# trflorian/s3od

Hardware: AMD Instinct MI355X
Metric: train images/sec (dinob 1024px bf16) at 1/2/4/8 GPU; infer masks/sec 1GPU (higher is better)
Workload: dtype bf16; 1 GPU; synth_sod train model=dinob 1024px bs=16/GPU fwd+focal_iou loss+bwd+AdamW; model=dinob (DINOv3 ViT-B/16 + DPT + 3-mask head), global_batch=16, image_size=1024, parallelism=dp1, rccl_world_size=1

## Files before the change

s3od_amd/csrc/gemm.hpp:

```cpp
#pragma once
#include "common.hpp"
#include <algorithm>

constexpr int GEMM_THREADS = 512;
constexpr int GEMM_WAVES = GEMM_THREADS / 64;
template <typename T> struct KT { static constexpr int BK = 64; };
template <> struct KT<float> { static constexpr int BK = 32; };

DEV int kc_off(int r, int byte) { return r * 128 + ((((byte >> 4) ^ ((r >> 1) & 7)) << 4) | (byte & 15)); }
template <int RB> DEV int mc_off(int k, int byte) {
  constexpr int SLOTS = RB / 32;
  int g = ((k & 3) | (((k >> 3) & 1) << 2)) & (SLOTS - 1);
  return k * RB + ((((byte >> 5) ^ g) << 5) | (byte & 31));
}

struct ConvGeo {
  int B;
  int SH, SW, SC;
  int RH, RW;
  int KH, KW, s, p;
  int py, px, kh0, kw0, nth, ntw, qy0, qx0;
};

static inline ConvGeo make_class(ConvGeo g, int OH, int OW, int py, int px) {
// ... 819 lines not shown
      }
    };
    const int spr_ = BN / 8;
    if (fixed_cols && BM % (NT / spr_) == 0) {
      const int rpi = NT / spr_, cs = tid % spr_, r0 = tid / spr_, n = n0 + cs * 8, nit = BM / rpi;
      if (n < N) {
        dispatch([&](auto ACTC) {
#pragma unroll
          for (int it0 = 0; it0 < nit; it0 += EB) {
            __builtin_amdgcn_sched_barrier(0);
            float av[EB][8];
            Row8<TR> q[EB];
            long orow[EB];
#pragma unroll
            for (int u = 0; u < EB; u++) {
              const int it = it0 + u, r = r0 + it * rpi, m = m0 + r;
              if (it < nit) {
                const float4* src = (const float4*)(ct + r * LDT + cs * 8);
                const float4 x0 = src[0], x1 = src[1];
                av[u][0] = x0.x; av[u][1] = x0.y; av[u][2] = x0.z; av[u][3] = x0.w;
                av[u][4] = x1.x; av[u][5] = x1.y; av[u][6] = x1.z; av[u][7] = x1.w;
                orow[u] = m < M ? rm.map(m) : 0;
                if (res1) q[u].load(res1 + orow[u] * ldr1 + n);
              }
            }
#pragma unroll
            for (int u = 0; u < EB; u++) {
              const int it = it0 + u;
              if (it < nit && m0 + r0 + it * rpi < M) {
                float r1v[8];
                q[u].get(r1v);
                seg(ACTC, orow[u], n, av[u], r1v, b8, s8, h8);
              }
            }
          }
        });
      }
    } else {
      dispatch([&](auto ACTC) {
        for_segments(ct, LDT, BM, BN, m0, n0, M, N, tid, NT, [&](int m, int n, const float* a, int, int) {
          float av[8], bb[8], ss[8], hh[8], r1v[8];
#pragma unroll
          for (int e = 0; e < 8; e++) {
            av[e] = a[e];
            bb[e] = bias ? bias[n + e] : 0.f; ss[e] = scale ? scale[n + e] : 1.f; hh[e] = shift ? shift[n + e] : 0.f;
            r1v[e] = 0.f;
          }
          const long orow = rm.map(m);
          if (res1) load8<TR>(res1 + orow * ldr1 + n, r1v);
          seg(ACTC, orow, n, av, r1v, bb, ss, hh);
        });
      });
    }
    if (stats) {
      const int nph = NT / BN;
      const int c = tid % BN, ph = tid / BN;
      const int n = n0 + c;
      if (n < N) {
        float s = 0.f, q = 0.f;
        const float bn_ = bias ? bias[n] : 0.f;
        for (int r = ph; r < BM; r += nph) {
          if (m0 + r >= M) break;
          const float v = ct[r * LDT + c] + bn_;
          s += v; q += v * v;
        }
        const int rep = (int)(((unsigned)(blockIdx.y * gridDim.x + blockIdx.x) * (unsigned)nph + ph + (m0 / BM)) % S3OD_NREP);
        double* st = stats + (long)rep * 2 * N;
        atomicAdd(st + n, (double)s);
        atomicAdd(st + N + n, (double)q);
      }
    }
    if (csum) {
      lds_barrier();
      float* red = (float*)ct;
#pragma unroll
      for (int e = 0; e < 8; e++) red[tid * 8 + e] = cs8[e];
      lds_barrier();
      const int spr = BN / 8, nph = NT / spr;
      if (tid < BN && n0 + tid < N) {
        const int g = tid >> 3, e = tid & 7;
        float s = 0.f;
        for (int ph = 0; ph < nph; ph++) s += red[(ph * spr + g) * 8 + e];
        atomicAdd(csum + n0 + tid, s);
      }
    }
  }
};

struct EpiWgrad {
  float* dw; int M, N, Cx, taps;
  DEV void prepare(int) {}
  DEV void operator()(const float* ct, int LDT, int m0, int n0, int tid, int BM, int BN, int NT) const {
    const int total = BM * BN;
    for (int s = tid; s < total; s += NT) {
      int r = s / BN, c = s - r * BN;
      int m = m0 + r, n = n0 + c;
      if (m < M && n < N) {
        int tap = n / Cx, cin = n - tap * Cx;
        atomicAdd(dw + ((long)m * Cx + cin) * taps + tap, ct[r * LDT + c]);
      }
    }
  }
};

struct EpiWgradPart {
  float* ws; int M, N;
  int z = 0;
  DEV void prepare(int zz) { z = zz; }
  DEV void operator()(const float* ct, int LDT, int m0, int n0, int tid, int BM, int BN, int NT) const {
    float* slab = ws + (long)z * M * N;
    for_segments(ct, LDT, BM, BN, m0, n0, M, N, tid, NT, [&](int m, int n, const float* a, int, int) {
      float4* d = (float4*)(slab + (long)m * N + n);
      d[0] = make_float4(a[0], a[1], a[2], a[3]);
      d[1] = make_float4(a[4], a[5], a[6], a[7]);
    });
  }
};

template <bool KCL> struct PPFrag;
template <> struct PPFrag<true> {
  int o[2];
  DEV void init(int lane, int) {
#pragma unroll
    for (int kk = 0; kk < 2; kk++) o[kk] = kc_off(lane & 15, kk * 64 + (lane >> 4) * 16);
  }
  DEV bf16x8 read(const char* img, int row0, int kk) const { return *(const bf16x8*)(img + o[kk] + row0 * 128); }
};
template <> struct PPFrag<false> {
  int base, gk;
  DEV void init(int lane, int h64) {
    const int g = lane >> 4, i = lane & 15, q = i >> 2, p = i & 3;
    base = (8 * g + q) * 256 + 8 * p; gk = (q | ((g & 1) << 2)) ^ (h64 << 2);
  }
  DEV bf16x8 read(const char* img, int row0, int kk) const {
    typedef __attribute__((address_space(3))) s16x4 lds_s4;
    const char* a = img + base + ((((row0 >> 4) ^ gk)) << 5) + kk * 8192;
    s16x4 lo = __builtin_amdgcn_ds_read_tr16_b64_v4i16((lds_s4*)a);
    s16x4 hi = __builtin_amdgcn_ds_read_tr16_b64_v4i16((lds_s4*)(a + 1024));
    bf16x4 x = __builtin_bit_cast(bf16x4, lo), y = __builtin_bit_cast(bf16x4, hi);
    bf16x8 r;
    r[0] = x[0]; r[1] = x[1]; r[2] = x[2]; r[3] = x[3]; r[4] = y[0]; r[5] = y[1]; r[6] = y[2]; r[7] = y[3];
    return r;
  }
};


#ifdef S3OD_TIMELINE
static __device__ unsigned long long* s3od_tl;
#define S3OD_TL(slot, v) do { if (s3od_tl && threadIdx.x == 0) s3od_tl[((long)blockIdx.z * gridDim.y * gridDim.x + \
    blockIdx.y * gridDim.x + blockIdx.x) * 8 + (slot)] = (v); } while (0)
#else
#define S3OD_TL(slot, v) do { } while (0)
#endif

DEV void tile_of_block(int G, int& mt, int& nt) {
  const int nN = gridDim.x, nM = gridDim.y, nwg = nN * nM;
  const int L = blockIdx.y * nN + blockIdx.x;
  const int q = nwg >> 3, r = nwg & 7, xcd = L & 7, idx = L >> 3;
  const int W = (xcd < r ? xcd * (q + 1) : r * (q + 1) + (xcd - r) * q) + idx;
  if (G <= 0) { mt = W / nN; nt = W % nN; return; }
  const int per = G * nN, g = W / per, w = W - g * per, m_first = g * G, gs = min(nM - m_first, G);
  mt = m_first + w % gs; nt = w / gs;
}

template <class LA, class LB, class EPI>
__global__ void __launch_bounds__(GEMM_THREADS, 1) igemm_pp_kernel(LA la0, LB lb0, EPI epi, int KTILES, int split, int flags) {
  typedef bf16 T;
  constexpr int BM = 256, BN = 256, HB = 128 * 128, STG = 4 * HB, LDT = BN + 4;
  static_assert(sizeof(T) == 2 && KT<T>::BK == 64, "ping-pong kernel is bf16 only");
  static_assert(128 * LDT * 4 <= 160 * 1024 && 2 * STG <= 128 * LDT * 4, "ping-pong LDS budget");
  extern __shared__ __attribute__((aligned(16))) char smem[];
  const int tid = threadIdx.x, lane = tid & 63, wave = wave_id();
  const int wr = wave >> 2, wc = wave & 3;
  S3OD_TL(0, __builtin_amdgcn_s_memrealtime());
  S3OD_TL(3, ((unsigned long long)__builtin_amdgcn_s_getreg((20 << 0) | (0 << 6) | (31 << 11)) << 32) |
             (unsigned)__builtin_amdgcn_s_getreg((4 << 0) | (0 << 6) | (31 << 11)));
  int m0, n0;
  {
    int mt, nt_;
    tile_of_block((flags >> 8) & 0xff, mt, nt_);
    m0 = mt * BM; n0 = nt_ * BN;
  }
  const int per = (KTILES + split - 1) / split;
  const int kt0 = blockIdx.z * per, kt1 = min(KTILES, kt0 + per);
  const int nt = kt1 - kt0;
  epi.prepare(blockIdx.z);
  LA la1 = la0; LB lb1 = lb0;
  la0.setup(m0, tid); la1.setup(m0 + 128, tid);
  lb0.setup(n0, tid); lb1.setup(n0 + 128, tid);
  constexpr int NA = LA::NIW * 2;
  const bool stag = !(flags & 1);
  f32x4 acc[8][4];
#pragma unroll
  for (int i = 0; i < 8; i++)
#pragma unroll
    for (int j = 0; j < 4; j++) acc[i][j] = f32x4{0.f, 0.f, 0.f, 0.f};
  if (nt > 0) {
    la0.issue(kt0, smem); la1.issue(kt0, smem + HB); lb0.issue(kt0, smem + 2 * HB); lb1.issue(kt0, smem + 3 * HB);
    if (nt > 1) { la0.issue(kt0 + 1, smem + STG); la1.issue(kt0 + 1, smem + STG + HB); wait_vmcnt<NA>(); }
    else wait_vmcnt<0>();
    raw_barrier();
    if (wr && stag) raw_barrier();
    PPFrag<LA::KCL> pfa; pfa.init(lane, 0);
    PPFrag<LB::KCL> pfb; pfb.init(lane, wc & 1);
    const int boff = LB::KCL ? (wc & 1) * 64 * 128 : 0;
    bf16x8 fa[2][4][2], fb[2][2][2];
    auto rdA = [&](const char* As, int qm) {
#pragma unroll
      for (int i = 0; i < 4; i++)
#pragma unroll
        for (int kk = 0; kk < 2; kk++) {
          fa[qm][i][kk] = pfa.read(As, qm * 64 + i * 16, kk);
          if constexpr (LA::RELU) fa[qm][i][kk] = relu_frag(fa[qm][i][kk]);
        }
    };
    auto rdB = [&](const char* Bs, int qn) {
#pragma unroll
      for (int j = 0; j < 2; j++)
#pragma unroll
        for (int kk = 0; kk < 2; kk++) {
          fb[qn][j][kk] = pfb.read(Bs, qn * 32 + j * 16, kk);
          if constexpr (LB::RELU) fb[qn][j][kk] = relu_frag(fb[qn][j][kk]);
        }
    };
    auto mm = [&](int qm, int qn) {
      raw_barrier();
      wait_lgkm0();
      __builtin_amdgcn_s_setprio(1);
#pragma unroll
      for (int kk = 0; kk < 2; kk++)
#pragma unroll
        for (int i = 0; i < 4; i++)
#pragma unroll
          for (int j = 0; j < 2; j++)
            acc[qm * 4 + i][qn * 2 + j] =
                __builtin_amdgcn_mfma_f32_16x16x32_bf16(fb[qn][j][kk], fa[qm][i][kk], acc[qm * 4 + i][qn * 2 + j], 0, 0, 0);
      __builtin_amdgcn_s_setprio(0);
      raw_barrier();
    };
    for (int t = 0; t < nt; ++t) {
      char* cb = smem + (t & 1) * STG;
      char* nb = smem + ((t + 1) & 1) * STG;
      const char* As = cb + wr * HB;
      const char* Bs = cb + (2 + (wc >> 1)) * HB + boff;
      rdA(As, 0); rdB(Bs, 0);
      if (t + 1 < nt) lb0.issue(kt0 + t + 1, nb + 2 * HB);
      mm(0, 0);
      rdB(Bs, 1); rdA(As, 1);
      if (t + 1 < nt) lb1.issue(kt0 + t + 1, nb + 3 * HB);
      mm(0, 1);
      if (t + 2 < nt) la0.issue(kt0 + t + 2, cb);
      mm(1, 1);
      if (t + 2 < nt) { la1.issue(kt0 + t + 2, cb + HB); wait_vmcnt<NA>(); }
      else if (t + 1 < nt) wait_vmcnt<0>();
      mm(1, 0);
    }
    if (!wr && stag) raw_barrier();
  }
  S3OD_TL(1, __builtin_amdgcn_s_memrealtime());
  vm_drain();
  float* ct0 = (float*)smem;
  float* ct1 = ct0 + 64 * LDT;
  auto round = [&](auto CC) {
    constexpr int c = decltype(CC)::value;
    lds_barrier();
    {
      float* dst = wr ? ct1 : ct0;
#pragma unroll
      for (int i = 0; i < 4; i++)
#pragma unroll
        for (int j = 0; j < 4; j++) {
          const int r = i * 16 + (lane & 15), col = wc * 64 + j * 16 + (lane >> 4) * 4;
          *(f32x4*)(dst + r * LDT + col) = acc[c * 4 + i][j];
        }
    }
    lds_barrier();
    S3OD_TL(4 + 2 * c, __builtin_amdgcn_s_memrealtime());
#ifdef S3OD_TIMELINE
    if constexpr (std::is_same_v<EPI, EpiStd<bf16, bf16, bf16>>) {
      if (flags & 2) {
        const int cs = tid % 32, r0 = tid / 32;
#pragma unroll
        for (int it = 0; it < 8; it++) {
          const int r = r0 + (it & 3) * 16;
          const float* src_ = (it < 4 ? ct0 : ct1) + r * LDT + cs * 8;
          const float4 a = ((const float4*)src_)[0], b = ((const float4*)src_)[1];
          const float v[8] = {a.x, a.y, a.z, a.w, b.x, b.y, b.z, b.w};
          store8<bf16>(epi.out + (long)(m0 + (it < 4 ? 0 : 128) + c * 64 + r) * epi.ldo + n0 + cs * 8, v);
        }
        return;
      }
    }
#endif
    epi(ct0, LDT, m0 + c * 64, n0, tid, 64, BN, GEMM_THREADS);
    epi(ct1, LDT, m0 + 128 + c * 64, n0, tid, 64, BN, GEMM_THREADS);
    if (c == 0) S3OD_TL(5, __builtin_amdgcn_s_memrealtime());
  };
  round(std::integral_constant<int, 0>{});
  round(std::integral_constant<int, 1>{});
  S3OD_TL(2, __builtin_amdgcn_s_memrealtime());
}
constexpr int PP_LDS = 128 * (256 + 4) * 4;

template <class LA, class LB, class EPI>
int launch_igemm_q(LA la, LB lb, EPI epi, int M, int N, int KTILES, int split, int zdim_extra, hipStream_t st);

template <typename T, int BM, int BN, class LA, class LB, class EPI, int NST = 3, int WM_ = 0>
static int launch_igemm(LA la, LB lb, EPI epi, int M, int N, int KTILES, int split, int zdim_extra, hipStream_t st) {
  if constexpr (WM_ < 0) {
    static_assert(BM == 256 && BN == 256 && sizeof(T) == 2, "q config");
    return launch_igemm_q(la, lb, epi, M, N, KTILES, split, zdim_extra, st);
  } else if constexpr (LA::ROWS * 2 == BM) {
    static_assert(BM == 256 && BN == 256 && LB::ROWS == 128 && sizeof(T) == 2, "ping-pong config");
    if (!la.buf_ok() || !lb.buf_ok()) {
      s3od_set_error("igemm: operand window too large for a buffer descriptor or gather channels < %d", KT<T>::BK / 2);
      return 22;
    }
    auto kfn = igemm_pp_kernel<LA, LB, EPI>;
    static const bool attr = ((void)hipFuncSetAttribute((const void*)kfn, hipFuncAttributeMaxDynamicSharedMemorySize, PP_LDS), true);
    (void)attr;
    const int flags = S3OD_KNOB("S3OD_PP_FLAGS", 0) | (S3OD_KNOB("S3OD_GEMM_GROUP", 0) & 0xff) << 8;
    dim3 grid(cdiv(N, BN), cdiv(M, BM), split * zdim_extra);
    hipLaunchKernelGGL(kfn, grid, dim3(GEMM_THREADS), PP_LDS, st, la, lb, epi, KTILES, split, flags);
    return s3od_check_launch("igemm_pp");
  } else {
    if (!la.buf_ok() || !lb.buf_ok()) {
      s3od_set_error("igemm: operand window too large for a buffer descriptor or gather channels < %d", KT<T>::BK / 2);
      return 22;
    }
    typedef GemmShape<T, BM, BN, NST, WM_> S;
    auto kfn = igemm_kernel<T, BM, BN, NST, LA, LB, EPI, WM_>;
    static const bool attr = ((void)hipFuncSetAttribute((const void*)kfn, hipFuncAttributeMaxDynamicSharedMemorySize, S::LDS), true);
    (void)attr;
    dim3 grid(cdiv(N, BN), cdiv(M, BM), split * zdim_extra);
    hipLaunchKernelGGL(kfn, grid, dim3(GEMM_THREADS), S::LDS, st, la, lb, epi, KTILES, split);
    return s3od_check_launch("igemm");
  }
}
```

s3od_amd/csrc/gemm_q.hip:

```cpp
#include "gemm.hpp"

namespace {
constexpr int Q_THREADS = 256, Q_BM = 256, Q_BN = 256, Q_STAGE = (Q_BM + Q_BN) * 128, Q_LDT = Q_BN + 4;
constexpr int Q_LDS = (2 * Q_STAGE > 128 * Q_LDT * 4) ? 2 * Q_STAGE : 128 * Q_LDT * 4;
static_assert(Q_LDS <= 160 * 1024, "q kernel LDS budget");
}

DEV void q_wait_lgkm0() { __builtin_amdgcn_s_waitcnt(0xC07F); }

template <class LA, class LB, class EPI>
__global__ void __launch_bounds__(Q_THREADS, 1) igemm_q_kernel(LA la, LB lb, EPI epi, int KTILES, int split, int group) {
  typedef bf16 T;
  static_assert(LA::ROWS == 256 && LB::ROWS == 256 && LA::NIW == 8 && LB::NIW == 8, "q kernel: 256-row loaders on 4 waves");
  extern __shared__ __attribute__((aligned(16))) char smem[];
  const int tid = threadIdx.x, lane = tid & 63, wave = wave_id();
  const int wm = wave >> 1, wn = wave & 1;
  int m0, n0;
  {
    int mt, nt_;
    tile_of_block(group, mt, nt_);
    m0 = mt * Q_BM; n0 = nt_ * Q_BN;
  }
  const int per = (KTILES + split - 1) / split;
  const int kt0 = blockIdx.z * per, kt1 = min(KTILES, kt0 + per);
  const int nt = kt1 - kt0;
  epi.prepare(blockIdx.z);
  la.setup(m0, tid);
  lb.setup(n0, tid);
  constexpr int NL = LA::NIW + LB::NIW;
  f32x4 acc[8][8];
#pragma unroll
  for (int i = 0; i < 8; i++)
#pragma unroll
    for (int j = 0; j < 8; j++) acc[i][j] = f32x4{0.f, 0.f, 0.f, 0.f};
  bf16x8 fa[2][8], fb[2][8];
  auto read_frags = [&](int buf, const char* stage, int kk) {
#pragma unroll
    for (int i = 0; i < 8; i++) fa[buf][i] = Frag<T, LA::KCL, Q_BM>::read(stage, wm * 128 + i * 16, kk, lane);
#pragma unroll
    for (int j = 0; j < 8; j++) fb[buf][j] = Frag<T, LB::KCL, Q_BN>::read(stage + Q_BM * 128, wn * 128 + j * 16, kk, lane);
  };
  auto mfmas = [&](int buf) {
    if constexpr (LA::RELU) {
#pragma unroll
      for (int i = 0; i < 8; i++) fa[buf][i] = relu_frag(fa[buf][i]);
    }
    if constexpr (LB::RELU) {
#pragma unroll
      for (int j = 0; j < 8; j++) fb[buf][j] = relu_frag(fb[buf][j]);
    }
    asm volatile("s_nop 1");
#pragma unroll
    for (int i = 0; i < 8; i++)
#pragma unroll
      for (int j = 0; j < 8; j++)
        asm volatile("v_mfma_f32_16x16x32_bf16 %0, %1, %2, %0" : "+a"(acc[i][j]) : "v"(fb[buf][j]), "v"(fa[buf][i]));
    asm volatile("s_nop 7\n\ts_nop 7" :: "v"(fa[buf][0]), "v"(fa[buf][1]), "v"(fa[buf][2]), "v"(fa[buf][3]),
                 "v"(fa[buf][4]), "v"(fa[buf][5]), "v"(fa[buf][6]), "v"(fa[buf][7]), "v"(fb[buf][0]), "v"(fb[buf][1]),
                 "v"(fb[buf][2]), "v"(fb[buf][3]), "v"(fb[buf][4]), "v"(fb[buf][5]), "v"(fb[buf][6]), "v"(fb[buf][7]));
  };
  auto issue = [&](int kt, char* stage) {
    la.issue(kt, stage);
    lb.issue(kt, stage + Q_BM * 128);
  };
  if (nt > 0) {
    issue(kt0, smem);
    if (nt > 1) { issue(kt0 + 1, smem + Q_STAGE); wait_vmcnt<NL>(); }
    else wait_vmcnt<0>();
    raw_barrier();
    read_frags(0, smem, 0);
    for (int t = 0; t + 1 < nt; ++t) {
      char* cur = smem + (t & 1) * Q_STAGE;
      char* nxt = smem + ((t + 1) & 1) * Q_STAGE;
      q_wait_lgkm0();
      read_frags(1, cur, 1);
      mfmas(0);
      wait_vmcnt<0>();
      q_wait_lgkm0();
      raw_barrier();
      if (t + 2 < nt) issue(kt0 + t + 2, cur);
      read_frags(0, nxt, 0);
      mfmas(1);
    }
    q_wait_lgkm0();
    read_frags(1, smem + ((nt - 1) & 1) * Q_STAGE, 1);
    mfmas(0);
    mfmas(1);
  }
  asm volatile("s_nop 7\n\ts_nop 7\n\ts_nop 7" ::: "memory");
  vm_drain();
  float* ct = (float*)smem;
#pragma unroll
  for (int h = 0; h < 2; h++) {
    lds_barrier();
    if (wm == h) {
#pragma unroll
      for (int i = 0; i < 8; i++)
#pragma unroll
        for (int j = 0; j < 8; j++) {
          const int r = i * 16 + (lane & 15), c = wn * 128 + j * 16 + (lane >> 4) * 4;
          *(f32x4*)(ct + r * Q_LDT + c) = acc[i][j];
        }
    }
    lds_barrier();
    epi(ct, Q_LDT, m0 + h * 128, n0, tid, 128, Q_BN, Q_THREADS);
  }
}

template <class LA, class LB, class EPI>
int launch_igemm_q(LA la, LB lb, EPI epi, int M, int N, int KTILES, int split, int zdim_extra, hipStream_t st) {
  if (!la.buf_ok() || !lb.buf_ok()) {
    s3od_set_error("igemm_q: operand window too large for a buffer descriptor");
    return 22;
  }
  auto kfn = igemm_q_kernel<LA, LB, EPI>;
  static const bool attr = ((void)hipFuncSetAttribute((const void*)kfn, hipFuncAttributeMaxDynamicSharedMemorySize, Q_LDS), true);
  (void)attr;
  dim3 grid(cdiv(N, Q_BN), cdiv(M, Q_BM), split * zdim_extra);
  const int group = S3OD_KNOB("S3OD_GEMM_GROUP", 0);
  hipLaunchKernelGGL(kfn, grid, dim3(Q_THREADS), Q_LDS, st, la, lb, epi, KTILES, split, group);
  return s3od_check_launch("igemm_q");
}

typedef DenseKC<bf16, 256, 4> QKC;
typedef DenseMC<bf16, 256, 4> QMC;
template int launch_igemm_q<QKC, QKC, EpiStd<bf16, bf16, bf16>>(QKC, QKC, EpiStd<bf16, bf16, bf16>, int, int, int, int, int, hipStream_t);
template int launch_igemm_q<QKC, QKC, EpiStd<float, float, bf16>>(QKC, QKC, EpiStd<float, float, bf16>, int, int, int, int, int, hipStream_t);
template int launch_igemm_q<QKC, QKC, EpiStd<float, bf16, bf16>>(QKC, QKC, EpiStd<float, bf16, bf16>, int, int, int, int, int, hipStream_t);
template int launch_igemm_q<QKC, QKC, EpiStd<bf16, float, bf16>>(QKC, QKC, EpiStd<bf16, float, bf16>, int, int, int, int, int, hipStream_t);
template int launch_igemm_q<QKC, QMC, EpiStd<bf16, bf16, bf16>>(QKC, QMC, EpiStd<bf16, bf16, bf16>, int, int, int, int, int, hipStream_t);
template int launch_igemm_q<QKC, QMC, EpiStd<float, float, float>>(QKC, QMC, EpiStd<float, float, float>, int, int, int, int, int, hipStream_t);
template int launch_igemm_q<QMC, QMC, EpiWgradPart>(QMC, QMC, EpiWgradPart, int, int, int, int, int, hipStream_t);
template int launch_igemm_q<QMC, QMC, EpiWgrad>(QMC, QMC, EpiWgrad, int, int, int, int, int, hipStream_t);
```

s3od_amd/csrc/linear_ops.hip:

```cpp
#include "gemm_dispatch.hpp"
int blaslt_gemm_rm(const void* A, long lda, const void* B, long ldb, const void* C, long ldc, void* D, long ldd, int M,
                   int N, int K, hipStream_t st);

template <typename T> struct EpiQKV {
  T* q; T* k; T* v; const float* bias; const float* cs; const float* sn;
  int M, Ntok, P, H;
  int moff = 0;
  DEV void prepare(int) {}
  DEV void operator()(const float* ct, int LDT, int m0, int n0, int tid, int BM, int BN, int NT) const {
    float b8[8], bp8[8];
    {
      const int nn = n0 + (tid % (BN / 8)) * 8, dd = nn & 63, dc = dd < 32 ? 32 : -32;
#pragma unroll
      for (int e = 0; e < 8; e++) { b8[e] = bias ? bias[nn + e] : 0.f; bp8[e] = bias ? bias[nn + dc + e] : 0.f; }
    }
    const bool fixed_cols = NT % (BN / 8) == 0;
    for_segments(ct, LDT, BM, BN, m0, n0, M, 3 * H * 64, tid, NT, [&](int m, int n, const float* a, int r, int c) {
      int which = n / (H * 64), nn = n - which * H * 64, h = nn >> 6, d0 = nn & 63;
      int b = (m + moff) / Ntok, t = (m + moff) - b * Ntok;
      float val[8];
#pragma unroll
      for (int e = 0; e < 8; e++) val[e] = a[e] + (fixed_cols ? b8[e] : (bias ? bias[n + e] : 0.f));
      if (which < 2 && t >= Ntok - P) {
        int dc = d0 < 32 ? 32 : -32;
        const float4* pa = (const float4*)(ct + r * LDT + c + dc);
        float4 p0 = pa[0], p1 = pa[1];
        float pv[8] = {p0.x, p0.y, p0.z, p0.w, p1.x, p1.y, p1.z, p1.w};
        int tp = t - (Ntok - P);
        const float4* cr = (const float4*)(cs + (long)tp * 64 + d0);
        const float4* sr = (const float4*)(sn + (long)tp * 64 + d0);
        float4 c0 = cr[0], c1 = cr[1], s0 = sr[0], s1 = sr[1];
        float cv[8] = {c0.x, c0.y, c0.z, c0.w, c1.x, c1.y, c1.z, c1.w};
        float sv[8] = {s0.x, s0.y, s0.z, s0.w, s1.x, s1.y, s1.z, s1.w};
#pragma unroll
        for (int e = 0; e < 8; e++) {
          float q = pv[e] + (fixed_cols ? bp8[e] : (bias ? bias[n + dc + e] : 0.f));
          float rot = d0 < 32 ? -q : q;
          val[e] = val[e] * cv[e] + rot * sv[e];
        }
      }
      if (which == 0) {
#pragma unroll
        for (int e = 0; e < 8; e++) val[e] *= S3OD_QSCALE;
      }
      T* dst = which == 0 ? q : (which == 1 ? k : v);
      store8<T>(dst + (((long)b * H + h) * Ntok + t) * 64 + d0, val);
    });
  }
};

template <class F> static int for_row_panels(int M, int row_mode, F f) {
  if (!(row_mode == 0 && M > 256 && (M & 255) != 0)) return f(0, M, false);
  const int M1 = M & ~255;
  if (int rc = f(0, M1, false)) return rc;
  return f(M1, M - M1, true);
}

template <bool BKC, int U, class EPI>
__global__ void __launch_bounds__(256) tail_gemm_kernel(const bf16* __restrict__ A, long lda, const bf16* __restrict__ Bp,
                                                        long ldb, int M, int N, int K, EPI epi) {
  constexpr int LDT = 64 + 4;
  __shared__ __attribute__((aligned(16))) float ct[2048];
  const int tid = threadIdx.x, lane = tid & 63, wave = tid >> 6, g = lane >> 4, l = lane & 15;
  const int m0 = blockIdx.y * 16, nb0 = blockIdx.x * 64, am = m0 + l, bn = nb0 + wave * 16 + l;
  const bool aok = am < M, bok = bn < N;
  const bf16* ar = A + (long)(aok ? am : 0) * lda;
  const long bo = bok ? bn : 0;
  f32x4 acc = {0.f, 0.f, 0.f, 0.f};
  constexpr int RS = 24;
  static_assert(sizeof(float) * 2048 + (BKC ? 2 : 2 * 4 * U * 32 * RS) <= 160 * 1024, "tail_gemm: LDS budget (gfx950: 160 KiB)");
  __shared__ bf16 bst[BKC ? 1 : 4 * U * 32 * RS];
  bf16* wst = bst + (BKC ? 0 : wave * U * 32 * RS);
  const int bj = lane >> 1, bc = 8 * (lane & 1);
  const long bcol = (nb0 + wave * 16 + bc < N) ? nb0 + wave * 16 + bc : 0;
  auto load = [&](int k, bf16x8& fa, bf16x8& fb) {
    fa = *(const bf16x8*)(ar + k);
    if constexpr (BKC) fb = *(const bf16x8*)(Bp + bo * ldb + k);
  };
  const int KF = K / 32;
  int kk = 0;
  for (; kk + U <= KF; kk += U) {
    bf16x8 fa[U], fb[U];
    uint4 braw[BKC ? 1 : U];
#pragma unroll
    for (int u = 0; u < U; u++) {
      load((kk + u) * 32 + 8 * g, fa[u], fb[u]);
      if constexpr (!BKC) braw[u] = *(const uint4*)(Bp + (long)((kk + u) * 32 + bj) * ldb + bcol);
    }
    if constexpr (!BKC) {
      __builtin_amdgcn_fence(__ATOMIC_RELEASE, "wavefront");
      __builtin_amdgcn_wave_barrier();
#pragma unroll
      for (int u = 0; u < U; u++) *(uint4*)(wst + (u * 32 + bj) * RS + bc) = braw[u];
      __builtin_amdgcn_fence(__ATOMIC_ACQ_REL, "wavefront");
      __builtin_amdgcn_wave_barrier();
#pragma unroll
      for (int u = 0; u < U; u++)
#pragma unroll
        for (int e = 0; e < 8; e++) fb[u][e] = wst[(u * 32 + 8 * g + e) * RS + l];
    }
    __builtin_amdgcn_sched_barrier(0);
#pragma unroll
    for (int u = 0; u < U; u++) acc = __builtin_amdgcn_mfma_f32_16x16x32_bf16(fb[u], fa[u], acc, 0, 0, 0);
  }
  for (; kk < KF; kk++) {
    bf16x8 fa, fb;
    load(kk * 32 + 8 * g, fa, fb);
    if constexpr (!BKC) {
#pragma unroll
      for (int e = 0; e < 8; e++) fb[e] = Bp[(long)(kk * 32 + 8 * g + e) * ldb + bo];
    }
    acc = __builtin_amdgcn_mfma_f32_16x16x32_bf16(fb, fa, acc, 0, 0, 0);
  }
  if (K % 32) {
    bf16x8 fa, fb;
    const int k = KF * 32 + 8 * g;
    if (k < K) {
      load(k, fa, fb);
      if constexpr (!BKC) {
#pragma unroll
        for (int e = 0; e < 8; e++) fb[e] = Bp[(long)(k + e) * ldb + bo];
      }
    } else {
#pragma unroll
      for (int e = 0; e < 8; e++) { fa[e] = (bf16)0.f; fb[e] = (bf16)0.f; }
    }
    acc = __builtin_amdgcn_mfma_f32_16x16x32_bf16(fb, fa, acc, 0, 0, 0);
  }
  *(f32x4*)(ct + l * LDT + wave * 16 + 4 * g) = acc;
  __syncthreads();
  epi.prepare(0);
  epi(ct, LDT, m0, nb0, tid, 16, 64, 256);
}
template <class LA, class LB, class EPI>
static int launch_tail_gemm(const LA& la, const LB& lb, EPI e, int M, int N, hipStream_t st) {
  const int KF = la.K / 32;
  auto go = [&](auto u) {
    hipLaunchKernelGGL((tail_gemm_kernel<LB::KCL, decltype(u)::value, EPI>), dim3(cdiv(N, 64), cdiv(M, 16)), dim3(256), 0, st,
                       (const bf16*)la.p, la.ld, (const bf16*)lb.p, lb.ld, M, N, la.K, e);
    return s3od_check_launch("igemm tail");
  };
  if constexpr (LB::KCL) {
    if (KF % 24 == 0) return go(std::integral_constant<int, 24>{});
    if (KF % 16 == 0) return go(std::integral_constant<int, 16>{});
  } else {
    if (KF % 16 == 0) return go(std::integral_constant<int, 16>{});
    if (KF % 12 == 0) return go(std::integral_constant<int, 12>{});
  }
  return go(std::integral_constant<int, 8>{});
}
template <typename T, class C, class LA, class LB, class EPI>
static int launch_op(LA la, LB lb, EPI e, int M, int N, int KTILES, bool tail, hipStream_t st) {
  if constexpr (!C::PP && sizeof(T) == 2 && LA::KCL)
    if (tail && !la.relu && !lb.relu && !S3OD_OFF("S3OD_TAIL_SKINNY"))
      return launch_tail_gemm(la, lb, e, M, N, st);
  return launch_igemm<T, C::BM, C::BN, LA, LB, EPI, C::NST, C::WM>(la, lb, e, M, N, KTILES, 1, 1, st);
}

static int linear_fwd_rows(int dtype, int M, int N, int K, const void* x, long ldx, const void* w,
                           const float* bias, const float* scale, const float* shift, int act,
                           const void* res1, long ldr1, const void* res2, long ldr2, int res_f32,
                           void* out, long ldo, int out_f32, void* pre, long ldp,
                           int row_mode, int P, int prefix, bool tail, void* stream) {
  RowMap rm = dense_rm(); rm.mode = row_mode; rm.P = P; rm.prefix = prefix;
  hipStream_t st = (hipStream_t)stream;
  DISPATCH_T(dtype, {
    const int KTILES = cdiv(K, KT<T>::BK);
    auto go = [&](auto tile, auto tout, auto tres) -> int {
      typedef decltype(tout) TO; typedef decltype(tres) TR;
      const int def = (pp_pays(M, N) && N % 256 == 0) ? 5 : (K >= 2048 ? 0 : 1);
      return with_cfg<T, true>(def, tail, [&](auto C) -> int {
        DenseKC<T, decltype(C)::LM, decltype(C)::W> la{(const T*)x, ldx, M, K, 0};
        DenseKC<T, decltype(C)::LN, decltype(C)::W> lb{(const T*)w, (long)K, N, K, 0};
        EpiStd<TO, TR, T> e{(TO*)out, ldo, 0, bias, scale, shift, (const TR*)res1, ldr1, (const TR*)res2, ldr2,
                            (T*)pre, ldp, nullptr, act, M, N, rm};
        return launch_op<T, decltype(C)>(la, lb, e, M, N, KTILES, tail, st);
      });
    };
    if (out_f32 && res_f32) return go(0, float{}, float{});
    if (out_f32) return go(0, float{}, T{});
    if (res_f32) return go(0, T{}, float{});
    return go(0, T{}, T{});
  });
  return 0;
}

static int linear_dgrad_rows(int dtype, int M, int N, int K, const void* dy, long lddy, const void* w,
                             int act, const void* aux, long ldaux, void* dx, long lddx, int out_f32,
                             int row_mode, int P, int prefix, float* colsum, bool tail, void* stream) {
  if (!tail && dtype == S3OD_BF16 && act == ACT_NONE && !out_f32 && row_mode == 0 && !colsum &&
      S3OD_KNOB("S3OD_DGRAD_BLASLT", 1) &&
      blaslt_gemm_rm(dy, lddy, w, N, aux, ldaux, dx, lddx, M, N, K, (hipStream_t)stream) == 0)
    return s3od_check_launch("linear_dgrad (hipBLASLt)");
  RowMap rm = dense_rm(); rm.mode = row_mode; rm.P = P; rm.prefix = prefix;
  hipStream_t st = (hipStream_t)stream;
  DISPATCH_T(dtype, {
    const int KTILES = cdiv(K, KT<T>::BK);
    const int def = (pp_pays(M, N) && N % 256 == 0 && (K >= 2048 || act != ACT_NONE)) ? 5 : 1;
    return with_cfg<T, true>(def, tail, [&](auto C) -> int {
      DenseKC<T, decltype(C)::LM, decltype(C)::W> la{(const T*)dy, lddy, M, K, 0};
      DenseMC<T, decltype(C)::LN, decltype(C)::W> lb{(const T*)w, (long)N, K, N};
      if (out_f32) {
        EpiStd<float, float> e{(float*)dx, lddx, 0, nullptr, nullptr, nullptr, (const float*)aux, ldaux, nullptr, 0, nullptr, 0, nullptr, act, M, N, rm, colsum};
        return launch_op<T, decltype(C)>(la, lb, e, M, N, KTILES, tail, st);
      }
      EpiStd<T, T> e{(T*)dx, lddx, 0, nullptr, nullptr, nullptr, (const T*)aux, ldaux, nullptr, 0, nullptr, 0, nullptr, act, M, N, rm, colsum};
      return launch_op<T, decltype(C)>(la, lb, e, M, N, KTILES, tail, st);
    });
  });
  return 0;
}

template <typename T, class F> static int linear_wgrad_route(int Nout, int Kin, int rows, int split, F f) {
  const int def = (long)Nout * Kin > 1024L * 1024 ? 5 : 0;
  return with_cfg<T, true>(def, false, [&](auto C) -> int {
    typedef decltype(C) CC;
    const int KTILES = cdiv(rows, KT<T>::BK);
    const int sp = split > 0 ? split : wgrad_split<T, CC::BM, CC::BN, CC::NST>(cdiv(Nout, CC::BM) * cdiv(Kin, CC::BN), KTILES);
    const bool slabs = CC::SLAB && slab_ok() && Kin % 4 == 0 && sp > 1;
    return f(C, sp, slabs ? (long)sp * Nout * Kin : 0L);
  });
}

extern "C" {

#ifdef S3OD_TIMELINE
int s3od_dbg_timeline(unsigned long long* buf) {
  return hipMemcpyToSymbol(HIP_SYMBOL(s3od_tl), &buf, sizeof(buf)) == hipSuccess ? 0 : 1;
}
#endif

int s3od_linear_fwd(int dtype, int M, int N, int K, const void* x, long ldx, const void* w,
                    const float* bias, const float* scale, const float* shift, int act,
                    const void* res1, long ldr1, const void* res2, long ldr2, int res_f32,
                    void* out, long ldo, int out_f32, void* pre, long ldp,
                    int row_mode, int P, int prefix, void* stream) {
  S3OD_REQUIRE(K % 8 == 0 && N % 8 == 0, "linear_fwd: K and N must be multiples of 8 (K=%d N=%d)", K, N);
  const long es = dtype == S3OD_BF16 ? 2 : 4, eo = out_f32 ? 4 : es, er = res_f32 ? 4 : es;
  return for_row_panels(M, row_mode, [&](int m0, int rows, bool tail) -> int {
    return linear_fwd_rows(dtype, rows, N, K, (const char*)x + m0 * ldx * es, ldx, w, bias, scale, shift, act,
                           res1 ? (const char*)res1 + m0 * ldr1 * er : nullptr, ldr1,
                           res2 ? (const char*)res2 + m0 * ldr2 * er : nullptr, ldr2, res_f32,
                           (char*)out + m0 * ldo * eo, ldo, out_f32, pre ? (char*)pre + m0 * ldp * es : nullptr, ldp,
                           row_mode, P, prefix, tail, stream);
  });
}

int s3od_linear_dgrad(int dtype, int M, int N, int K, const void* dy, long lddy, const void* w,
                      int act, const void* aux, long ldaux, void* dx, long lddx, int out_f32,
                      int row_mode, int P, int prefix, float* colsum, void* stream) {
  S3OD_REQUIRE(K % 8 == 0 && N % 8 == 0, "linear_dgrad: K,N %% 8");
  const long es = dtype == S3OD_BF16 ? 2 : 4, eo = out_f32 ? 4 : es;
  return for_row_panels(M, row_mode, [&](int m0, int rows, bool tail) -> int {
    return linear_dgrad_rows(dtype, rows, N, K, (const char*)dy + m0 * lddy * es, lddy, w, act,
                             aux ? (const char*)aux + m0 * ldaux * eo : nullptr, ldaux, (char*)dx + m0 * lddx * eo, lddx,
                             out_f32, row_mode, P, prefix, colsum, tail, stream);
  });
}

int s3od_linear_wgrad_ws(int dtype, int Nout, int Kin, int rows, int split, long* bytes) {
  S3OD_REQUIRE(bytes != nullptr, "linear_wgrad_ws: null output");
  *bytes = 0;
  if (dtype != S3OD_BF16) return 0;
  return linear_wgrad_route<bf16>(Nout, Kin, rows, split, [&](auto, int, long slab_floats) -> int {
    *bytes = 4 * slab_floats;
    return 0;
  });
}

int s3od_linear_wgrad(int dtype, int Nout, int Kin, int rows, const void* dy, long lddy,
                      const void* x, long ldx, float* dw, int split, float* slab, long slab_bytes, void* stream) {
  S3OD_REQUIRE(Nout % 8 == 0 && Kin % 8 == 0, "linear_wgrad: dims %% 8");
  hipStream_t st = (hipStream_t)stream;
  DISPATCH_T(dtype, {
    const int KTILES = cdiv(rows, KT<T>::BK);
    return linear_wgrad_route<T>(Nout, Kin, rows, split, [&](auto C, int sp, long slab_floats) -> int {
      constexpr int BM = decltype(C)::BM, BN = decltype(C)::BN, NST = decltype(C)::NST;
      DenseMC<T, decltype(C)::LM, decltype(C)::W> la{(const T*)dy, lddy, rows, Nout};
      DenseMC<T, decltype(C)::LN, decltype(C)::W> lb{(const T*)x, ldx, rows, Kin};
      if constexpr (decltype(C)::SLAB) {
        if (slab && slab_floats > 0 && slab_bytes >= 4 * slab_floats) {
          EpiWgradPart e{slab, Nout, Kin};
          int rc = launch_igemm<T, BM, BN, decltype(la), decltype(lb), decltype(e), NST, decltype(C)::WM>(la, lb, e, Nout, Kin, KTILES, sp, 1, st);
          if (rc) return rc;
          hipLaunchKernelGGL(wgrad_reduce_kernel, dim3(cdiv((long)Nout * Kin / 4, 256)), dim3(256), 0, st, slab, sp, Nout, Kin, dw, Kin, 1);
          return s3od_check_launch("linear_wgrad reduce");
        }
      }
      EpiWgrad e{dw, Nout, Kin, Kin, 1};
      return launch_igemm<T, BM, BN, decltype(la), decltype(lb), decltype(e), NST, decltype(C)::WM>(la, lb, e, Nout, Kin, KTILES, sp, 1, st);
    });
  });
  return 0;
}

int s3od_qkv_rope_fwd(int dtype, int B, int Ntok, int P, int H, const void* x, const void* w, const float* bias,
                      const float* cos_t, const float* sin_t, void* q, void* k, void* v, void* stream) {
  const int D = 64 * H, N = 3 * D;
  hipStream_t st = (hipStream_t)stream;
  DISPATCH_T(dtype, {
    return for_row_panels(B * Ntok, 0, [&](int m_first, int M, bool tail) -> int {
      return with_cfg<T>(pp_pays(M, N) ? 5 : 1, tail, [&](auto C) -> int {
        DenseKC<T, decltype(C)::LM, decltype(C)::W> la{(const T*)x + (long)m_first * D, (long)D, M, D, 0};
        DenseKC<T, decltype(C)::LN, decltype(C)::W> lb{(const T*)w, (long)D, N, D, 0};
        EpiQKV<T> e{(T*)q, (T*)k, (T*)v, bias, cos_t, sin_t, M, Ntok, P, H};
        e.moff = m_first;
        return launch_op<T, decltype(C)>(la, lb, e, M, N, cdiv(D, KT<T>::BK), tail, st);
      });
    });
  });
  return 0;
}

}
```

Measured before the change: 111.8 images/s.

## Rewrite q GEMM kernel with 4-deep LDS ring and interleaved DMA/MFMA schedule

```diff
diff --git a/s3od_amd/csrc/gemm.hpp b/s3od_amd/csrc/gemm.hpp
--- a/s3od_amd/csrc/gemm.hpp
+++ b/s3od_amd/csrc/gemm.hpp
@@ -1145,6 +1145,94 @@
 }
 constexpr int PP_LDS = 128 * (256 + 4) * 4;
 
+DEV int kc64_x(int r) { const int h = (r >> 2) & 3; return h ^ ((h & 1) << 1); }
+typedef __attribute__((address_space(3))) const char lds_cchar;
+DEV unsigned lds_addr(const char* p) { return (unsigned)(unsigned long)(lds_cchar*)p; }
+DEV const char* lds_ptr(unsigned a) { return (const char*)(lds_cchar*)(unsigned long)a; }
+typedef int i32x4_t __attribute__((ext_vector_type(4)));
+DEV i32x4_t q_rsrc(const void* p, unsigned long bytes) {
+  const unsigned long a = (unsigned long)p;
+  return i32x4_t{(int)(unsigned)a, (int)((a >> 32) & 0xffff), (int)(unsigned)(bytes < BUF_MAX ? bytes : BUF_MAX), 0x00020000};
+}
+DEV void blds16s(i32x4_t r, unsigned voff, unsigned soff, unsigned lds_wave_base) {
+  asm volatile("s_mov_b32 m0, %3\n\ts_nop 0\n\tbuffer_load_dwordx4 %0, %1, %2 offen lds"
+               :: "v"(voff), "s"(r), "s"(soff), "s"(lds_wave_base) : "memory");
+}
+template <class L, bool KCL = L::KCL> struct KStep;
+template <class L> struct KStep<L, true> {
+  const bf16* pb; unsigned long nb; unsigned vo[4], vt[4]; int wb, klim, kpart;
+  DEV void setup(const L& l, int t0, int tid, int klim_) {
+    const int lane = tid & 63, wave = wave_id(), rem = l.nrows - t0;
+    wb = wave * 4096;
+    klim = klim_;
+    kpart = (klim & 31) ? klim >> 5 : -1;
+    pb = l.p + (long)t0 * l.ld;
+    nb = rem > 0 ? ((unsigned long)(min(rem, 256) - 1) * l.ld + l.K) * 2 : 0;
+    const int kel = ((lane & 3) ^ kc64_x(lane >> 2)) * 8;
+#pragma unroll
+    for (int i = 0; i < 4; i++) {
+      const int r = (wave * 4 + i) * 16 + (lane >> 2);
+      vo[i] = r < rem ? (unsigned)(((long)r * l.ld + kel) * 2) : BUF_OOB;
+      vt[i] = (klim & ~31) + kel < klim ? vo[i] : BUF_OOB;
+    }
+  }
+  DEV void piece(const L&, int ks, char* img, int i) const {
+    const auto rs = q_rsrc(pb, ks * 32 < klim ? nb : 0);
+    blds16s(rs, ks == kpart ? vt[i] : vo[i], (unsigned)ks * 64u, lds_addr(img) + wb + i * 1024);
+  }
+};
+template <class L> struct KStep<L, false> {
+  unsigned vo[4]; int wb; unsigned long tot;
+  DEV void setup(const L& l, int t0, int tid, int klim) {
+    const int lane = tid & 63, wave = wave_id();
+    wb = wave * 4096;
+    tot = klim > 0 ? ((unsigned long)(klim - 1) * l.ld + l.ncols) * 2 : 0;
+#pragma unroll
+    for (int i = 0; i < 4; i++) {
+      const int k = wave * 8 + (lane >> 5) + 2 * i;
+      const int cl = t0 + mc_logical_byte<512>(k, (lane & 31) * 16) / 2;
+      vo[i] = cl < l.ncols ? (unsigned)(((long)k * l.ld + cl) * 2) : BUF_OOB;
+    }
+  }
+  DEV void piece(const L& l, int ks, char* img, int i) const {
+    const unsigned long e0 = (unsigned long)ks * 32 * l.ld * 2;
+    const auto rs = q_rsrc((const char*)l.p + e0, e0 < tot ? tot - e0 : 0);
+    blds16s(rs, vo[i], 0u, lds_addr(img) + wb + i * 1024);
+  }
+};
+template <bool KCL> struct QFrag;
+template <> struct QFrag<true> {
+  unsigned a;
+  DEV void init(const char* img, int lane, int half) {
+    const int l = lane & 15;
+    a = lds_addr(img) + half * 8192 + l * 64 + (((lane >> 4) ^ kc64_x(l)) << 4);
+  }
+  DEV void flip(int d) { a += d; }
+  DEV bf16x8 read(int st01, int i) const { return *(const bf16x8*)(lds_ptr(a) + st01 * 32768 + i * 1024); }
+};
+template <> struct QFrag<false> {
+  unsigned a[8];
+  DEV void init(const char* img, int lane, int half) {
+    const int g = lane >> 4, l = lane & 15, q = l >> 2, p = l & 3, gk = q | ((g & 1) << 2);
+#pragma unroll
+    for (int i = 0; i < 8; i++) a[i] = lds_addr(img) + (8 * g + q) * 512 + half * 256 + ((i ^ gk) << 5) + 8 * p;
+  }
+  DEV void flip(int d) {
+#pragma unroll
+    for (int i = 0; i < 8; i++) a[i] += d;
+  }
+  DEV bf16x8 read(int st01, int i) const {
+    typedef __attribute__((address_space(3))) s16x4 lds_s4;
+    const char* s = lds_ptr(a[i]) + st01 * 32768;
+    s16x4 lo = __builtin_amdgcn_ds_read_tr16_b64_v4i16((lds_s4*)s);
+    s16x4 hi = __builtin_amdgcn_ds_read_tr16_b64_v4i16((lds_s4*)(s + 2048));
+    bf16x4 x = __builtin_bit_cast(bf16x4, lo), y = __builtin_bit_cast(bf16x4, hi);
+    bf16x8 r;
+    r[0] = x[0]; r[1] = x[1]; r[2] = x[2]; r[3] = x[3]; r[4] = y[0]; r[5] = y[1]; r[6] = y[2]; r[7] = y[3];
+    return r;
+  }
+};
+
 template <class LA, class LB, class EPI>
 int launch_igemm_q(LA la, LB lb, EPI epi, int M, int N, int KTILES, int split, int zdim_extra, hipStream_t st);
 
diff --git a/s3od_amd/csrc/gemm_q.hip b/s3od_amd/csrc/gemm_q.hip
--- a/s3od_amd/csrc/gemm_q.hip
+++ b/s3od_amd/csrc/gemm_q.hip
@@ -1,17 +1,20 @@
 #include "gemm.hpp"
 
 namespace {
-constexpr int Q_THREADS = 256, Q_BM = 256, Q_BN = 256, Q_STAGE = (Q_BM + Q_BN) * 128, Q_LDT = Q_BN + 4;
-constexpr int Q_LDS = (2 * Q_STAGE > 128 * Q_LDT * 4) ? 2 * Q_STAGE : 128 * Q_LDT * 4;
+constexpr int Q_THREADS = 256, Q_BM = 256, Q_BN = 256, Q_IMG = 256 * 64, Q_STAGE = 2 * Q_IMG, Q_RING = 4, Q_LDT = Q_BN + 4;
+constexpr int Q_LDS = (Q_RING * Q_STAGE > 128 * Q_LDT * 4) ? Q_RING * Q_STAGE : 128 * Q_LDT * 4;
 static_assert(Q_LDS <= 160 * 1024, "q kernel LDS budget");
+template <int V> using IC = std::integral_constant<int, V>;
+template <class F, int... I> DEV void q_seq(F& f, std::integer_sequence<int, I...>) { (f(IC<I>{}), ...); }
+template <int N, class F> DEV void q_for(F f) { q_seq(f, std::make_integer_sequence<int, N>{}); }
 }
 
 DEV void q_wait_lgkm0() { __builtin_amdgcn_s_waitcnt(0xC07F); }
 
 template <class LA, class LB, class EPI>
 __global__ void __launch_bounds__(Q_THREADS, 1) igemm_q_kernel(LA la, LB lb, EPI epi, int KTILES, int split, int group) {
-  typedef bf16 T;
   static_assert(LA::ROWS == 256 && LB::ROWS == 256 && LA::NIW == 8 && LB::NIW == 8, "q kernel: 256-row loaders on 4 waves");
+  static_assert(!LA::RELU && !LB::RELU, "q kernel: no ReLU-on-load (a VALU write of a fragment inside the MFMA stream)");
   extern __shared__ __attribute__((aligned(16))) char smem[];
   const int tid = threadIdx.x, lane = tid & 63, wave = wave_id();
   const int wm = wave >> 1, wn = wave & 1;
@@ -23,69 +26,67 @@
   }
   const int per = (KTILES + split - 1) / split;
   const int kt0 = blockIdx.z * per, kt1 = min(KTILES, kt0 + per);
-  const int nt = kt1 - kt0;
+  const int ks0 = 2 * kt0, n = 2 * (kt1 - kt0);
   epi.prepare(blockIdx.z);
-  la.setup(m0, tid);
-  lb.setup(n0, tid);
-  constexpr int NL = LA::NIW + LB::NIW;
+  const int klim = min(la.K, (ks0 + n) * 32);
+  KStep<LA> sa; KStep<LB> sb;
+  sa.setup(la, m0, tid, klim);
+  sb.setup(lb, n0, tid, klim);
+  QFrag<LA::KCL> qa; QFrag<LB::KCL> qb;
+  qa.init(smem, lane, wm);
+  qb.init(smem + Q_IMG, lane, wn);
   f32x4 acc[8][8];
 #pragma unroll
   for (int i = 0; i < 8; i++)
 #pragma unroll
     for (int j = 0; j < 8; j++) acc[i][j] = f32x4{0.f, 0.f, 0.f, 0.f};
   bf16x8 fa[2][8], fb[2][8];
-  auto read_frags = [&](int buf, const char* stage, int kk) {
+  auto read_frag = [&](int buf, int st01, int f) {
+    if (f < 8) fb[buf][f] = qb.read(st01, f);
+    else fa[buf][f - 8] = qa.read(st01, f - 8);
+  };
+  auto dma_piece = [&](int ks, char* stage, int d) {
+    if (d < 4) sa.piece(la, ks, stage, d);
+    else sb.piece(lb, ks, stage + Q_IMG, d - 4);
+  };
+  constexpr int FPG = (LA::KCL || LB::KCL) ? 2 : 1;
+  constexpr int D0 = 4 + 16 / FPG + 4, DS = 4;
+  static_assert(D0 + 7 * DS < 64, "DMA pieces inside the block");
+  auto kstep = [&](auto PC, int ks, char* stage, int flip) __attribute__((always_inline)) {
+    constexpr int P = decltype(PC)::value;
+    if constexpr (P == 1) { qa.flip(flip); qb.flip(flip); }
+    q_wait_lgkm0();
+    asm volatile("s_nop 1");
+    q_for<64>([&](auto MC) __attribute__((always_inline)) {
+      constexpr int m = decltype(MC)::value, i = m >> 3, j = m & 7;
+      asm volatile("v_mfma_f32_16x16x32_bf16 %0, %1, %2, %0" : "+a"(acc[i][j]) : "v"(fb[P][j]), "v"(fa[P][i]));
+      if constexpr (m == 3) { wait_vmcnt<16>(); raw_barrier(); }
+      if constexpr (m >= 4 && m < 4 + 16 / FPG) {
 #pragma unroll
-    for (int i = 0; i < 8; i++) fa[buf][i] = Frag<T, LA::KCL, Q_BM>::read(stage, wm * 128 + i * 16, kk, lane);
+        for (int u = 0; u < FPG; u++) read_frag(P ^ 1, P ^ 1, (m - 4) * FPG + u);
+      }
+      if constexpr (m >= D0 && (m - D0) % DS == 0 && (m - D0) / DS < 8) dma_piece(ks + 4, stage, (m - D0) / DS);
+      __builtin_amdgcn_sched_barrier(0);
+    });
+    asm volatile("" :: "v"(fa[P][0]), "v"(fa[P][1]), "v"(fa[P][2]), "v"(fa[P][3]),
+                 "v"(fa[P][4]), "v"(fa[P][5]), "v"(fa[P][6]), "v"(fa[P][7]), "v"(fb[P][0]), "v"(fb[P][1]),
+                 "v"(fb[P][2]), "v"(fb[P][3]), "v"(fb[P][4]), "v"(fb[P][5]), "v"(fb[P][6]), "v"(fb[P][7]));
+  };
+  if (n > 0) {
 #pragma unroll
-    for (int j = 0; j < 8; j++) fb[buf][j] = Frag<T, LB::KCL, Q_BN>::read(stage + Q_BM * 128, wn * 128 + j * 16, kk, lane);
-  };
-  auto mfmas = [&](int buf) {
-    if constexpr (LA::RELU) {
+    for (int q = 0; q < Q_RING; q++)
 #pragma unroll
-      for (int i = 0; i < 8; i++) fa[buf][i] = relu_frag(fa[buf][i]);
+      for (int d = 0; d < 8; d++) dma_piece(ks0 + q, smem + q * Q_STAGE, d);
+    wait_vmcnt<24>();
+    raw_barrier();
+#pragma unroll
+    for (int f = 0; f < 16; f++) read_frag(0, 0, f);
+    int pair = 0, flip = 2 * Q_STAGE;
+    for (int s = 0; s < n; s += 2) {
+      kstep(IC<0>{}, ks0 + s, smem + pair, flip);
+      kstep(IC<1>{}, ks0 + s + 1, smem + pair + Q_STAGE, flip);
+      pair ^= 2 * Q_STAGE; flip = -flip;
     }
-    if constexpr (LB::RELU) {
-#pragma unroll
-      for (int j = 0; j < 8; j++) fb[buf][j] = relu_frag(fb[buf][j]);
-    }
-    asm volatile("s_nop 1");
-#pragma unroll
-    for (int i = 0; i < 8; i++)
-#pragma unroll
-      for (int j = 0; j < 8; j++)
-        asm volatile("v_mfma_f32_16x16x32_bf16 %0, %1, %2, %0" : "+a"(acc[i][j]) : "v"(fb[buf][j]), "v"(fa[buf][i]));
-    asm volatile("s_nop 7\n\ts_nop 7" :: "v"(fa[buf][0]), "v"(fa[buf][1]), "v"(fa[buf][2]), "v"(fa[buf][3]),
-                 "v"(fa[buf][4]), "v"(fa[buf][5]), "v"(fa[buf][6]), "v"(fa[buf][7]), "v"(fb[buf][0]), "v"(fb[buf][1]),
-                 "v"(fb[buf][2]), "v"(fb[buf][3]), "v"(fb[buf][4]), "v"(fb[buf][5]), "v"(fb[buf][6]), "v"(fb[buf][7]));
-  };
-  auto issue = [&](int kt, char* stage) {
-    la.issue(kt, stage);
-    lb.issue(kt, stage + Q_BM * 128);
-  };
-  if (nt > 0) {
-    issue(kt0, smem);
-    if (nt > 1) { issue(kt0 + 1, smem + Q_STAGE); wait_vmcnt<NL>(); }
-    else wait_vmcnt<0>();
-    raw_barrier();
-    read_frags(0, smem, 0);
-    for (int t = 0; t + 1 < nt; ++t) {
-      char* cur = smem + (t & 1) * Q_STAGE;
-      char* nxt = smem + ((t + 1) & 1) * Q_STAGE;
-      q_wait_lgkm0();
-      read_frags(1, cur, 1);
-      mfmas(0);
-      wait_vmcnt<0>();
-      q_wait_lgkm0();
-      raw_barrier();
-      if (t + 2 < nt) issue(kt0 + t + 2, cur);
-      read_frags(0, nxt, 0);
-      mfmas(1);
-    }
-    q_wait_lgkm0();
-    read_frags(1, smem + ((nt - 1) & 1) * Q_STAGE, 1);
-    mfmas(0);
-    mfmas(1);
   }
   asm volatile("s_nop 7\n\ts_nop 7\n\ts_nop 7" ::: "memory");
   vm_drain();
diff --git a/s3od_amd/csrc/linear_ops.hip b/s3od_amd/csrc/linear_ops.hip
--- a/s3od_amd/csrc/linear_ops.hip
+++ b/s3od_amd/csrc/linear_ops.hip
@@ -212,7 +212,7 @@
 }
 
 template <typename T, class F> static int linear_wgrad_route(int Nout, int Kin, int rows, int split, F f) {
-  const int def = (long)Nout * Kin > 1024L * 1024 ? 5 : 0;
+  const int def = (long)Nout * Kin > 1024L * 1024 ? 6 : 0;
   return with_cfg<T, true>(def, false, [&](auto C) -> int {
     typedef decltype(C) CC;
     const int KTILES = cdiv(rows, KT<T>::BK);
```

New measurement: 114.5 images/s (median of 6 runs). +2.4%, better.
